# TonyLianLong/LLM-groundedDiffusion

Hardware: AMD Instinct MI355X
Metric: images/sec (50-step SD1.5 512^2, LMD+ guidance) (higher is better)
Workload: dtype fp16; 1 GPU; LMD+ stage 2, 4 cached 2-box layouts/GPU/step (lmd_v0.1 cache), 50 DDIM steps, 512x512, sd14_gligen (SD1.4+GLIGEN architecture, seeded random weights), VAE decodes included; per-box masks = box masks; mask_refinement=box, layouts_per_gpu=4, num_inference_steps=50, parallelism=dp1, rccl_ranks=1, lanes_per_gpu=4, gemm_tuning=throughput

## Files before the change

llm-groundeddiffusion_amd/csrc/gemm.hip:

```cpp
#include "common.h"
#include "../../include/lgd_hip.h"
#include <map>
#include <mutex>
#include <utility>
#include <stdlib.h>

namespace {

constexpr int BK = 64;
constexpr int LDS_LD = BK + 16;

struct GemmArgs {
  LgdGemmDesc d;
  int cin;
  int k_per_split;
  int group_m;
#ifdef LGD_GEMM_ABLATION
  int stagger;
#endif
};

__device__ __forceinline__ float4 ld_bias4(const float* p, int n) {
  return *reinterpret_cast<const float4*>(p + n);
}

__device__ __forceinline__ f32x4 rownorm4(const LgdGemmDesc& d, int m, int n_in, f32x4 v) {
  if (d.epi & LGD_EPI_ROWNORM) {
    const float2 st = *reinterpret_cast<const float2*>(d.rowstat + (long)m * 2);
    const float4 cs = *reinterpret_cast<const float4*>(d.colsum + n_in);
    v[0] = st.y * (v[0] - st.x * cs.x); v[1] = st.y * (v[1] - st.x * cs.y);
    v[2] = st.y * (v[2] - st.x * cs.z); v[3] = st.y * (v[3] - st.x * cs.w);
  }
  return v;
}

template <bool GEGLU>
__device__ __forceinline__ f32x4 epilogue_value4(const LgdGemmDesc& d, long r_off, int m, int n_out, f32x4 v, f32x4 g,
                                                 float4 bv, float4 bg, bool res_ready, half4_t res_pre) {
  v[0] += bv.x; v[1] += bv.y; v[2] += bv.z; v[3] += bv.w;
  if (GEGLU) {
    g[0] += bg.x; g[1] += bg.y; g[2] += bg.z; g[3] += bg.w;
#ifdef LGD_GEMM_ABLATION
    if (d.epi & (1 << 16)) {
#pragma unroll
      for (int r = 0; r < 4; ++r) v[r] = v[r] * g[r];
    } else
#endif
    {
      const f32x2_t g01 = gelu2_f((f32x2_t){g[0], g[1]}), g23 = gelu2_f((f32x2_t){g[2], g[3]});
      v[0] *= g01[0]; v[1] *= g01[1]; v[2] *= g23[0]; v[3] *= g23[1];
    }
  }
  const float alpha = d.alpha;
#pragma unroll
  for (int r = 0; r < 4; ++r) v[r] *= alpha;
  if (res_ready) {
#pragma unroll
    for (int r = 0; r < 4; ++r) v[r] += (float)res_pre[r];
  } else if (d.res) {
    if (d.epi & LGD_EPI_RES_F32) {
      const float* rp = reinterpret_cast<const float*>(d.res) + r_off + (long)m * d.ldr + n_out;
      float4 rv = *reinterpret_cast<const float4*>(rp);
      v[0] += rv.x; v[1] += rv.y; v[2] += rv.z; v[3] += rv.w;
    } else {
      const half_t* rp = reinterpret_cast<const half_t*>(d.res) + r_off + (long)m * d.ldr + n_out;
      half4_t rv = *reinterpret_cast<const half4_t*>(rp);
#pragma unroll
      for (int r = 0; r < 4; ++r) v[r] += (float)rv[r];
    }
  }
  return v;
}

template <bool GEGLU>
__device__ __forceinline__ void epilogue_store4(const LgdGemmDesc& d, long c_off, long r_off, int m,
                                                int n_out, f32x4 v, f32x4 g, float4 bv, float4 bg,
                                                bool res_ready = false,
                                                half4_t res_pre = (half4_t){0, 0, 0, 0}) {
  v = epilogue_value4<GEGLU>(d, r_off, m, n_out, v, g, bv, bg, res_ready, res_pre);
  if (d.epi & LGD_EPI_OUT_F32) {
    float* cp = reinterpret_cast<float*>(d.c) + c_off + (long)m * d.ldc + n_out;
    *reinterpret_cast<float4*>(cp) = make_float4(v[0], v[1], v[2], v[3]);
  } else {
    half_t* cp = reinterpret_cast<half_t*>(d.c) + c_off + (long)m * d.ldc + n_out;
    half4_t o;
#pragma unroll
    for (int r = 0; r < 4; ++r) o[r] = (half_t)v[r];
    *reinterpret_cast<half4_t*>(cp) = o;
  }
}

__device__ __forceinline__ float4 ld_bias_sum4(const LgdGemmDesc& d, int n) {
  float4 b = make_float4(0.f, 0.f, 0.f, 0.f);
  if (d.bias) b = ld_bias4(d.bias, n);
  if (d.bias2) {
    float4 b2 = ld_bias4(d.bias2, n);
    b.x += b2.x; b.y += b2.y; b.z += b2.z; b.w += b2.w;
  }
  return b;
}

template <int MI, int NI>
__device__ __forceinline__ void gemm_epilogue(const GemmArgs& ga, f32x4 (&acc)[NI][MI], int m0, int n0,
                                              int wm, int wn, int lane, int batch, int split,
                                              long c_off, long r_off, int* lds_flag = nullptr) {
  const LgdGemmDesc& d = ga.d;
  const int m_l = lane & 15;
  const int n_l = (lane >> 4) * 4;
  if (d.splits > 1) {
    float* ws = ga.d.ws + ((long)batch * d.splits + split) * (long)d.M * d.N;
#pragma unroll
    for (int mi = 0; mi < MI; ++mi) {
      int m = m0 + wm * 16 * MI + mi * 16 + m_l;
      if (m >= d.M) continue;
#pragma unroll
      for (int ni = 0; ni < NI; ++ni) {
        int n = n0 + wn * 16 * NI + ni * 16 + n_l;
        if (n >= d.N) continue;
        f32x4 v = acc[ni][mi];
        *reinterpret_cast<float4*>(ws + (long)m * d.N + n) = make_float4(v[0], v[1], v[2], v[3]);
      }
    }
    if (!d.cnt || !lds_flag) return;
    asm volatile("s_waitcnt vmcnt(0)" ::: "memory");
    __syncthreads();
    int32_t* cnt = d.cnt + (long)batch * gridDim.x + blockIdx.x;
    if (threadIdx.x == 0) {
      __builtin_amdgcn_fence(__ATOMIC_RELEASE, "agent");
      asm volatile("s_waitcnt vmcnt(0)" ::: "memory");
      *lds_flag = __hip_atomic_fetch_add(cnt, 1, __ATOMIC_RELAXED, __HIP_MEMORY_SCOPE_AGENT);
    }
    __syncthreads();
    if (*lds_flag != d.splits - 1) return;
    if (threadIdx.x == 0) {
      __builtin_amdgcn_fence(__ATOMIC_ACQUIRE, "agent");
      __hip_atomic_store(cnt, 0, __ATOMIC_RELAXED, __HIP_MEMORY_SCOPE_AGENT);
    }
    __syncthreads();
    const float* w0 = ga.d.ws + (long)batch * d.splits * (long)d.M * d.N;
#pragma unroll
    for (int mi = 0; mi < MI; ++mi) {
      const int m = m0 + wm * 16 * MI + mi * 16 + m_l;
#pragma unroll
      for (int ni = 0; ni < NI; ++ni) {
        const int n = n0 + wn * 16 * NI + ni * 16 + n_l;
        f32x4 v = {0.f, 0.f, 0.f, 0.f};
        if (m < d.M && n < d.N) {
          for (int s2 = 0; s2 < d.splits; ++s2) {
            const float4 t = *reinterpret_cast<const float4*>(w0 + (long)s2 * d.M * d.N + (long)m * d.N + n);
            v[0] += t.x; v[1] += t.y; v[2] += t.z; v[3] += t.w;
          }
        }
        acc[ni][mi] = v;
      }
    }
  }
  const bool geglu = d.epi & LGD_EPI_GEGLU;
  if (geglu) {
// ... 48 lines not shown
        const int m = m0 + wm * 16 * MI + mi * 16 + m_l;
        if (m < d.M)
          epilogue_store4<false>(d, c_off, r_off, m, n, rownorm4(d, m, n, acc[ni][mi]), acc[ni][mi], bv, bv, res16,
                                 res16 ? rpre[nj][mi] : (half4_t){0, 0, 0, 0});
      }
    }
  }
}

template <int MI, int NI, int WM, int WN, int STAGE_B, bool GEGLU, bool RES_PREFETCH>
__device__ __forceinline__ void gemm_epilogue_lds_generic(const GemmArgs& ga, f32x4 (&acc)[NI][MI], int m0, int n0, int wm,
                                                  int wn, int lane, int tid, long c_off, long r_off,
                                                  unsigned char* lds) {
  const LgdGemmDesc& d = ga.d;
  constexpr int NT = 64 * WM * WN;
  constexpr int BM = WM * 16 * MI, BN = WN * 16 * NI;
  constexpr int BN_OUT = GEGLU ? BN / 2 : BN;
  constexpr int NI_OUT = GEGLU ? NI / 2 : NI;
  constexpr int CROW = BN_OUT * 2 + 16;
  constexpr int R = (BM * CROW <= STAGE_B) ? 1 : ((BM / 2) * CROW <= STAGE_B) ? 2 : 4;
  static_assert(MI % R == 0 && (BM / R) * CROW <= STAGE_B, "staged rows must fit one ring stage");
  constexpr int MI_R = MI / R;
  constexpr int WROWS = 16 * MI_R;
  constexpr int RROWS = WM * WROWS;
  constexpr int CPR = BN_OUT / 8;
  const int m_l = lane & 15, n_l = (lane >> 4) * 4;
  const int n0_out = GEGLU ? n0 / 2 : n0;
  const int n_total_out = GEGLU ? d.N / 2 : d.N;
  const bool res16 = d.res && !(d.epi & LGD_EPI_RES_F32);
  half_t* cbase = reinterpret_cast<half_t*>(d.c) + c_off;
  float4 bv[NI_OUT], bg[NI_OUT];
  const bool rn = d.epi & LGD_EPI_ROWNORM;
  float4 cv[NI_OUT], cg[NI_OUT];
  float2 st[MI];
#pragma unroll
  for (int no = 0; no < NI_OUT; ++no) {
    const int n_out = n0_out + wn * 16 * NI_OUT + no * 16 + n_l;
    const int n_in = GEGLU ? n0 + wn * 16 * NI + no * 32 + n_l : n_out;
    bv[no] = make_float4(0.f, 0.f, 0.f, 0.f);
    bg[no] = bv[no];
    cv[no] = bv[no];
    cg[no] = bv[no];
#ifdef LGD_GEMM_ABLATION
    if (d.epi & (1 << 18)) continue;
#endif
    if (n_out < n_total_out) {
      bv[no] = ld_bias_sum4(d, n_in);
      if (GEGLU && d.bias) bg[no] = ld_bias4(d.bias, n_in + 16);
      if (rn) {
        cv[no] = *reinterpret_cast<const float4*>(d.colsum + n_in);
        if (GEGLU) cg[no] = *reinterpret_cast<const float4*>(d.colsum + n_in + 16);
      }
    }
  }
#pragma unroll
  for (int mi = 0; mi < MI; ++mi) {
    int m = m0 + wm * 16 * MI + mi * 16 + m_l;
    if (m >= d.M) m = d.M - 1;
    st[mi] = rn ? *reinterpret_cast<const float2*>(d.rowstat + (long)m * 2) : make_float2(0.f, 1.f);
  }
  auto rownorm = [&](f32x4 v, const float2 s2, const float4 c) {
    if (rn) {
      v[0] = s2.y * (v[0] - s2.x * c.x); v[1] = s2.y * (v[1] - s2.x * c.y);
      v[2] = s2.y * (v[2] - s2.x * c.z); v[3] = s2.y * (v[3] - s2.x * c.w);
    }
    return v;
  };
#pragma unroll
  for (int r = 0; r < R; ++r) {
    half4_t rpre[NI_OUT][MI_R];
    if (res16 && !GEGLU) {
      const half_t* rb = reinterpret_cast<const half_t*>(d.res) + r_off;
#pragma unroll
      for (int no = 0; no < NI_OUT; ++no) {
        int n = n0_out + wn * 16 * NI_OUT + no * 16 + n_l;
        if (n >= n_total_out) n = 0;
#pragma unroll
        for (int mj = 0; mj < MI_R; ++mj) {
          int m = m0 + wm * 16 * MI + (r * MI_R + mj) * 16 + m_l;
          if (m >= d.M) m = d.M - 1;
          rpre[no][mj] = *reinterpret_cast<const half4_t*>(rb + (long)m * d.ldr + n);
        }
      }
    }
#pragma unroll
    for (int no = 0; no < NI_OUT; ++no) {
      const int n_out = n0_out + wn * 16 * NI_OUT + no * 16 + n_l;
      const int nn = n_out < n_total_out ? n_out : 0;
#pragma unroll
      for (int mj = 0; mj < MI_R; ++mj) {
        const int mi = r * MI_R + mj;
        int m = m0 + wm * 16 * MI + mi * 16 + m_l;
        if (m >= d.M) m = d.M - 1;
        f32x4 v;
        if constexpr (GEGLU) {
          v = epilogue_value4<true>(d, r_off, m, nn, rownorm(acc[2 * no][mi], st[mi], cv[no]), rownorm(acc[2 * no + 1][mi], st[mi], cg[no]),
                                    bv[no], bg[no], false, (half4_t){0, 0, 0, 0});
        } else {
          v = epilogue_value4<false>(d, r_off, m, nn, rownorm(acc[no][mi], st[mi], cv[no]), acc[no][mi], bv[no], bv[no], res16,
                                     res16 ? rpre[no][mj] : (half4_t){0, 0, 0, 0});
        }
        half4_t o;
#pragma unroll
        for (int e = 0; e < 4; ++e) o[e] = (half_t)v[e];
        *reinterpret_cast<half4_t*>(lds + (wm * WROWS + mj * 16 + m_l) * CROW + (wn * 16 * NI_OUT + no * 16 + n_l) * 2) = o;
      }
    }
    asm volatile("s_waitcnt lgkmcnt(0)" ::: "memory");
    __builtin_amdgcn_s_barrier();
#pragma unroll
    for (int i = 0; i < (RROWS * CPR + NT - 1) / NT; ++i) {
      const int idx = tid + i * NT;
      const int row = idx / CPR, ch = idx - row * CPR;
      const int wr = row / WROWS;
      const int m = m0 + wr * 16 * MI + r * WROWS + (row - wr * WROWS), n = n0_out + ch * 8;
#ifdef LGD_GEMM_ABLATION
      if ((d.epi & (1 << 17)) && idx != 0) continue;
#endif
      if (idx < RROWS * CPR && m < d.M && n < n_total_out) {
        const uint4 val = *reinterpret_cast<const uint4*>(lds + row * CROW + ch * 16);
        *reinterpret_cast<uint4*>(cbase + (long)m * d.ldc + n) = val;
      }
    }
    if (r + 1 < R || !RES_PREFETCH) {
      asm volatile("s_waitcnt lgkmcnt(0)" ::: "memory");
      __builtin_amdgcn_s_barrier();
    }
  }
}

template <int MI, int NI, int WM, int WN, int STAGE_B, bool GEGLU, bool RES_PREFETCH, bool RES16, bool RN>
__device__ __forceinline__ void gemm_epilogue_lds(const GemmArgs& ga, f32x4 (&acc)[NI][MI], int m0, int n0, int wm,
                                                  int wn, int lane, int tid, long c_off, long r_off,
                                                  unsigned char* lds) {
  static_assert(!(GEGLU && RES16), "GEGLU outputs take no residual here");
  const LgdGemmDesc& d = ga.d;
  constexpr int NT = 64 * WM * WN;
  constexpr int BM = WM * 16 * MI, BN = WN * 16 * NI;
  constexpr int BN_OUT = GEGLU ? BN / 2 : BN;
  constexpr int NI_OUT = GEGLU ? NI / 2 : NI;
  constexpr int CROW = BN_OUT * 2 + 16;
  constexpr int R = (BM * CROW <= STAGE_B) ? 1 : ((BM / 2) * CROW <= STAGE_B) ? 2 : 4;
  static_assert(MI % R == 0 && (BM / R) * CROW <= STAGE_B, "staged rows must fit one ring stage");
  constexpr int MI_R = MI / R;
  constexpr int WROWS = 16 * MI_R;
  constexpr int RROWS = WM * WROWS;
  constexpr int CPR = BN_OUT / 8;
  const int m_l = lane & 15, n_l = (lane >> 4) * 4;
  const int n0_out = GEGLU ? n0 / 2 : n0;
  const int n_total_out = GEGLU ? d.N / 2 : d.N;
  half_t* cbase = reinterpret_cast<half_t*>(d.c) + c_off;
  const f32x2_t alpha2 = {d.alpha, d.alpha};
  constexpr bool LEAN = MI * NI >= 32;
  constexpr bool LEAN2 = MI * NI >= 32 && WN == 4;
  float4 bv[NI_OUT], bg[NI_OUT], cv[NI_OUT], cg[NI_OUT];
  int ncol[NI_OUT];
#pragma unroll
  for (int no = 0; no < NI_OUT; ++no) {
    const int n_out = n0_out + wn * 16 * NI_OUT + no * 16 + n_l;
    const int n_in = GEGLU ? n0 + wn * 16 * NI + no * 32 + n_l : n_out;
    const bool ok = n_out < n_total_out;
    ncol[no] = ok ? n_out : 0;
    bv[no] = make_float4(0.f, 0.f, 0.f, 0.f);
    bg[no] = bv[no];
    cv[no] = bv[no];
    cg[no] = bv[no];
#ifdef LGD_GEMM_ABLATION
    if (d.epi & (1 << 18)) continue;
#endif
    if (ok && !LEAN2) {
      bv[no] = ld_bias_sum4(d, n_in);
      if (GEGLU && d.bias) bg[no] = ld_bias4(d.bias, n_in + 16);
      if constexpr (RN && !LEAN) {
        cv[no] = *reinterpret_cast<const float4*>(d.colsum + n_in);
        if (GEGLU) cg[no] = *reinterpret_cast<const float4*>(d.colsum + n_in + 16);
      }
    }
  }
  int mrow[MI];
  float2 st[MI];
#pragma unroll
  for (int mi = 0; mi < MI; ++mi) {
    int m = m0 + wm * 16 * MI + mi * 16 + m_l;
    if (m >= d.M) m = d.M - 1;
    mrow[mi] = m;
    st[mi] = make_float2(0.f, 1.f);
    if constexpr (RN && !LEAN2) st[mi] = *reinterpret_cast<const float2*>(d.rowstat + (long)m * 2);
  }
  auto normed = [&](const f32x4& v, const float2 s2, const float4 c, const float4 b, f32x2_t& lo, f32x2_t& hi) {
    lo = (f32x2_t){v[0], v[1]};
    hi = (f32x2_t){v[2], v[3]};
    if constexpr (RN) {
      const f32x2_t mean = {s2.x, s2.x}, rstd = {s2.y, s2.y};
      lo = rstd * (lo - mean * (f32x2_t){c.x, c.y});
      hi = rstd * (hi - mean * (f32x2_t){c.z, c.w});
    }
    lo += (f32x2_t){b.x, b.y};
    hi += (f32x2_t){b.z, b.w};
  };
  unsigned char* lw = lds + (wm * WROWS + m_l) * CROW + (wn * 16 * NI_OUT + n_l) * 2;
#pragma unroll
  for (int r = 0; r < R; ++r) {
    if constexpr (RN && LEAN2) {
#pragma unroll
      for (int mj = 0; mj < MI_R; ++mj)
        st[r * MI_R + mj] = *reinterpret_cast<const float2*>(d.rowstat + (long)mrow[r * MI_R + mj] * 2);
    }
    half4_t rpre[NI_OUT][MI_R];
    if constexpr (RES16) {
      const half_t* rb = reinterpret_cast<const half_t*>(d.res) + r_off;
#pragma unroll
      for (int mj = 0; mj < MI_R; ++mj) {
        const half_t* rrow = rb + (long)mrow[r * MI_R + mj] * d.ldr;
#pragma unroll
        for (int no = 0; no < NI_OUT; ++no) {
          int nc = ncol[no];
          if constexpr (LEAN) {
            const int n_out = n0_out + wn * 16 * NI_OUT + no * 16 + n_l;
            nc = n_out < n_total_out ? n_out : 0;
          }
          rpre[no][mj] = *reinterpret_cast<const half4_t*>(rrow + nc);
        }
      }
    }
#pragma unroll
    for (int no = 0; no < NI_OUT; ++no) {
      if constexpr ((RN && LEAN) || LEAN2) {
        const int n_out = n0_out + wn * 16 * NI_OUT + no * 16 + n_l;
        const int n_in = GEGLU ? n0 + wn * 16 * NI + no * 32 + n_l : n_out;
        if (n_out < n_total_out) {
          if constexpr (RN) {
            cv[no] = *reinterpret_cast<const float4*>(d.colsum + n_in);
            if (GEGLU) cg[no] = *reinterpret_cast<const float4*>(d.colsum + n_in + 16);
          }
          if constexpr (LEAN2) {
            bv[no] = ld_bias_sum4(d, n_in);
            if (GEGLU && d.bias) bg[no] = ld_bias4(d.bias, n_in + 16);
          }
        }
      }
#pragma unroll
      for (int mj = 0; mj < MI_R; ++mj) {
        const int mi = r * MI_R + mj;
        f32x2_t lo, hi;
        if constexpr (GEGLU) {
          f32x2_t glo, ghi;
          normed(acc[2 * no][mi], st[mi], cv[no], bv[no], lo, hi);
          normed(acc[2 * no + 1][mi], st[mi], cg[no], bg[no], glo, ghi);
#ifdef LGD_GEMM_ABLATION
          if (d.epi & (1 << 16)) { lo *= glo; hi *= ghi; } else
#endif
          { lo *= gelu2_f(glo); hi *= gelu2_f(ghi); }
        } else {
          normed(acc[no][mi], st[mi], cv[no], bv[no], lo, hi);
        }
        lo *= alpha2;
        hi *= alpha2;
        if constexpr (RES16) {
          const half4_t rr = rpre[no][mj];
          lo += (f32x2_t){(float)rr[0], (float)rr[1]};
          hi += (f32x2_t){(float)rr[2], (float)rr[3]};
        }
        const half4_t o = {(half_t)lo[0], (half_t)lo[1], (half_t)hi[0], (half_t)hi[1]};
        *reinterpret_cast<half4_t*>(lw + mj * 16 * CROW + no * 32) = o;
      }
    }
    asm volatile("s_waitcnt lgkmcnt(0)" ::: "memory");
    __builtin_amdgcn_s_barrier();
#pragma unroll LEAN2 ? 1 : (RROWS * CPR + NT - 1) / NT
    for (int i = 0; i < (RROWS * CPR + NT - 1) / NT; ++i) {
      const int idx = tid + i * NT;
      const int row = idx / CPR, ch = idx - row * CPR;
      const int wr = row / WROWS;
      const int m = m0 + wr * 16 * MI + r * WROWS + (row - wr * WROWS), n = n0_out + ch * 8;
#ifdef LGD_GEMM_ABLATION
      if ((d.epi & (1 << 17)) && idx != 0) continue;
#endif
      if (idx < RROWS * CPR && m < d.M && n < n_total_out) {
        const uint4 val = *reinterpret_cast<const uint4*>(lds + row * CROW + ch * 16);
        *reinterpret_cast<uint4*>(cbase + (long)m * d.ldc + n) = val;
      }
    }
    if (r + 1 < R || !RES_PREFETCH) {
      asm volatile("s_waitcnt lgkmcnt(0)" ::: "memory");
      __builtin_amdgcn_s_barrier();
    }
  }
}

template <int MI, int NI>
__global__ __launch_bounds__(256) void gemm_kernel(const GemmArgs ga) {
  constexpr int BM = 32 * MI;
  constexpr int BN = 32 * NI;
  constexpr int A_IT = BM * 8 / 256;
  constexpr int B_IT = BN * 8 / 256;
  static_assert(A_IT >= 1 && B_IT >= 1, "tile too small");

  __shared__ __attribute__((aligned(16))) half_t smem[(BM + BN) * LDS_LD];
  half_t* As = smem;
  half_t* Bs = smem + BM * LDS_LD;

  const LgdGemmDesc& d = ga.d;
  const int tid = threadIdx.x;
  const int lane = tid & 63;
  const int wid = tid >> 6;
  const int wm = wid >> 1, wn = wid & 1;

// ... 903 lines not shown
  const int frow = lane & 15, fg = lane >> 4, fsw = (frow >> 1) & 7;
  const unsigned lds0 = (unsigned)(uintptr_t)smem;
  unsigned a_ad0 = lds0 + (grp * 16 * MH + frow) * 128 + ((0 + fg) ^ fsw) * 16;
  unsigned a_ad1 = lds0 + (grp * 16 * MH + frow) * 128 + ((4 + fg) ^ fsw) * 16;
  unsigned b_ad0 = lds0 + OFF_B0 + (wn * 16 + frow) * 128 + ((0 + fg) ^ fsw) * 16;
  unsigned b_ad1 = lds0 + OFF_B0 + (wn * 16 + frow) * 128 + ((4 + fg) ^ fsw) * 16;
  using seqA = std::make_integer_sequence<int, MH>;
  using seqB0 = std::make_integer_sequence<int, NI0>;
  using seqB1 = std::make_integer_sequence<int, NI1>;

  f32x4 acc[NI][MI];
  half8_t af[2][MH], bf0[2][NI0], bf1[2][NI1];
  if constexpr (ABL & 2) {
#pragma unroll
    for (int kk = 0; kk < 2; ++kk) {
#pragma unroll
      for (int i = 0; i < MH; ++i) af[kk][i] = (half8_t){1, 1, 1, 1, 1, 1, 1, 1};
#pragma unroll
      for (int i = 0; i < NI0; ++i) bf0[kk][i] = (half8_t){1, 1, 1, 1, 1, 1, 1, 1};
#pragma unroll
      for (int i = 0; i < NI1; ++i) bf1[kk][i] = (half8_t){1, 1, 1, 1, 1, 1, 1, 1};
    }
  }

#define LGD_PH_MMA(BF, NB, NOFF, MOFF)                                                                              \
  {                                                                                                                 \
    asm volatile("s_waitcnt lgkmcnt(0)" ::: "memory");                                                              \
    __builtin_amdgcn_sched_barrier(0);                                                                              \
    if constexpr (!(ABL & 32)) __builtin_amdgcn_s_setprio(1);                                                       \
    _Pragma("unroll") for (int kk = 0; kk < 2; ++kk)                                                                \
      _Pragma("unroll") for (int ni = 0; ni < NB; ++ni)                                                             \
        _Pragma("unroll") for (int mi = 0; mi < MH; ++mi)                                                           \
          if constexpr (ABL & 4) asm volatile("" : "+v"(acc[NOFF + ni][MOFF + mi]) : "v"(BF[kk][ni]), "v"(af[kk][mi]));                \
          else acc[NOFF + ni][MOFF + mi] = __builtin_amdgcn_mfma_f32_16x16x32_f16(BF[kk][ni], af[kk][mi], acc[NOFF + ni][MOFF + mi], 0, 0, 0); \
    if constexpr (!(ABL & 32)) __builtin_amdgcn_s_setprio(0);                                                       \
    __builtin_amdgcn_sched_barrier(0);                                                                              \
  }
#define LGD_PH_BAR()                        \
  {                                         \
    __builtin_amdgcn_sched_barrier(0);      \
    __builtin_amdgcn_s_barrier();           \
    __builtin_amdgcn_sched_barrier(0);      \
  }

  if (nk > 0) {
    {
      unsigned sa, sw; int tap;
      k_pos(0, sa, sw, tap);
      dma_b(0, 0, true, sw, false);
      dma_a(0, 0, true, sa, tap, false);
      dma_b(1, 0, true, sw, false);
      dma_a(1, 0, true, sa, tap, false);
      k_pos(1, sa, sw, tap);
      dma_b(0, STAGE_B, nk > 1, sw, false);
      dma_a(0, STAGE_B, nk > 1, sa, tap, false);
    }
#pragma unroll
    for (int ni = 0; ni < NI; ++ni)
#pragma unroll
      for (int mi = 0; mi < MI; ++mi) acc[ni][mi] = (f32x4){0.f, 0.f, 0.f, 0.f};
    asm volatile("s_waitcnt vmcnt(%0)" ::"n"(T_DMA) : "memory");
    LGD_PH_BAR();
    if (grp == 1 && !(ABL & 64)) LGD_PH_BAR();
    unsigned so_cur = 0, so_nxt = STAGE_B;
    int sdelta = STAGE_B;
    for (int kt = 0; kt < nk; ++kt) {
      unsigned sa1, sw1, sa2, sw2; int tap1, tap2;
      k_pos(kt + 1, sa1, sw1, tap1);
      k_pos(kt + 2, sa2, sw2, tap2);
      const bool live1 = kt + 1 < nk, live2 = kt + 2 < nk;
      if constexpr (!(ABL & 2)) lds_read_frags<0, 64 * 128>(bf0[0], b_ad0, seqB0{});
      if constexpr (!(ABL & 2)) lds_read_frags<0, 64 * 128>(bf0[1], b_ad1, seqB0{});
      if constexpr (!(ABL & 2)) lds_read_frags<0, 16 * 128>(af[0], a_ad0, seqA{});
      if constexpr (!(ABL & 2)) lds_read_frags<0, 16 * 128>(af[1], a_ad1, seqA{});
      dma_b(1, so_nxt, live1, sw1);
      asm volatile("s_waitcnt vmcnt(%0)" ::"n"(T_DMA) : "memory");
      LGD_PH_BAR();
      LGD_PH_MMA(bf0, NI0, 0, 0);
      LGD_PH_BAR();
      if constexpr (!(ABL & 2)) lds_read_frags<BQ0_B, 64 * 128>(bf1[0], b_ad0, seqB1{});
      if constexpr (!(ABL & 2)) lds_read_frags<BQ0_B, 64 * 128>(bf1[1], b_ad1, seqB1{});
      dma_a(1, so_nxt, live1, sa1, tap1);
      asm volatile("s_waitcnt vmcnt(%0)" ::"n"(T_DMA) : "memory");
      LGD_PH_BAR();
      LGD_PH_MMA(bf1, NI1, NI0, 0);
      LGD_PH_BAR();
      if constexpr (!(ABL & 2)) lds_read_frags<OFF_A1, 16 * 128>(af[0], a_ad0, seqA{});
      if constexpr (!(ABL & 2)) lds_read_frags<OFF_A1, 16 * 128>(af[1], a_ad1, seqA{});
      dma_b(0, so_cur, live2, sw2);
      LGD_PH_BAR();
      LGD_PH_MMA(bf1, NI1, NI0, MH);
      LGD_PH_BAR();
      dma_a(0, so_cur, live2, sa2, tap2);
      asm volatile("s_waitcnt vmcnt(%0)" ::"n"(T_DMA) : "memory");
      LGD_PH_BAR();
      LGD_PH_MMA(bf0, NI0, 0, MH);
      LGD_PH_BAR();
      a_ad0 += sdelta; a_ad1 += sdelta; b_ad0 += sdelta; b_ad1 += sdelta;
      sdelta = -sdelta;
      const unsigned t = so_cur; so_cur = so_nxt; so_nxt = t;
    }
    if (grp == 0 && !(ABL & 64)) LGD_PH_BAR();
    asm volatile("s_waitcnt vmcnt(0) lgkmcnt(0)" ::: "memory");
    LGD_PH_BAR();
  }
  else {
#pragma unroll
    for (int ni = 0; ni < NI; ++ni)
#pragma unroll
      for (int mi = 0; mi < MI; ++mi) acc[ni][mi] = (f32x4){0.f, 0.f, 0.f, 0.f};
  }
#undef LGD_PH_MMA
#undef LGD_PH_BAR

  if constexpr (ABL & 16) {
#pragma unroll
    for (int ni = 0; ni < NI; ++ni)
#pragma unroll
      for (int mi = 0; mi < MI; ++mi) asm volatile("" ::"v"(acc[ni][mi]));
    return;
  }
  if (d.splits > 1) {
    const int m_l = lane & 15, n_l = (lane >> 4) * 4;
    float* ws = d.ws + ((long)batch * d.splits + split) * (long)d.M * d.N;
#pragma unroll
    for (int mi = 0; mi < MI; ++mi) {
      const int m = m0 + grp * 16 * MI + mi * 16 + m_l;
      if (m >= d.M) continue;
#pragma unroll
      for (int ni = 0; ni < NI; ++ni) {
        const int n = n0 + wn * 16 * NI + ni * 16 + n_l;
        if (n >= d.N) continue;
        const f32x4 v = acc[ni][mi];
        *reinterpret_cast<float4*>(ws + (long)m * d.N + n) = make_float4(v[0], v[1], v[2], v[3]);
      }
    }
    return;
  }
#define LGD_EPI_LDS(G, RS, RNORM) \
  gemm_epilogue_lds<MI, NI, WM, WN, (MI * NI > 32 ? STAGE_B : 2 * STAGE_B), G, true, RS, RNORM>(ga, acc, m0, n0, grp, wn, lane, tid, c_off, r_off, lds)
  const bool rn_ = d.epi & LGD_EPI_ROWNORM;
  if (d.epi & LGD_EPI_GEGLU) {
    if constexpr (NI % 2 == 0) {
      if (rn_) LGD_EPI_LDS(true, false, true); else LGD_EPI_LDS(true, false, false);
    }
  } else if (d.res) {
    if (rn_) LGD_EPI_LDS(false, true, true); else LGD_EPI_LDS(false, true, false);
  } else {
    if (rn_) LGD_EPI_LDS(false, false, true); else LGD_EPI_LDS(false, false, false);
  }
#undef LGD_EPI_LDS
}

__global__ __launch_bounds__(256) void splitk_reduce_kernel(const GemmArgs ga) {
  const LgdGemmDesc& d = ga.d;
  const bool geglu = d.epi & LGD_EPI_GEGLU;
  const int n_out_cols = geglu ? d.N / 2 : d.N;
  const long groups_per_row = n_out_cols / 4;
  const long total = (long)d.M * groups_per_row;
  const int batch = blockIdx.z;
  const int b_o = batch / d.nb_i, b_i = batch - b_o * d.nb_i;
  const long c_off = b_o * d.c_bs_o + b_i * d.c_bs_i;
  const long r_off = b_o * d.r_bs_o + b_i * d.r_bs_i;
  const float* ws = d.ws + (long)batch * d.splits * (long)d.M * d.N;
  for (long idx = blockIdx.x * 256L + threadIdx.x; idx < total; idx += (long)gridDim.x * 256L) {
    int m = (int)(idx / groups_per_row);
    int gcol = (int)(idx - (long)m * groups_per_row) * 4;
    int n_in = geglu ? (gcol / 16) * 32 + (gcol % 16) : gcol;
    f32x4 v = {0.f, 0.f, 0.f, 0.f}, g = {0.f, 0.f, 0.f, 0.f};
    for (int s = 0; s < d.splits; ++s) {
      const float* p = ws + (long)s * d.M * d.N + (long)m * d.N + n_in;
      float4 t = *reinterpret_cast<const float4*>(p);
      v[0] += t.x; v[1] += t.y; v[2] += t.z; v[3] += t.w;
      if (geglu) {
        float4 u = *reinterpret_cast<const float4*>(p + 16);
        g[0] += u.x; g[1] += u.y; g[2] += u.z; g[3] += u.w;
      }
    }
    const float4 bv = ld_bias_sum4(d, n_in);
    v = rownorm4(d, m, n_in, v);
    if (geglu) {
      float4 bg = make_float4(0.f, 0.f, 0.f, 0.f);
      if (d.bias) bg = ld_bias4(d.bias, n_in + 16);
      epilogue_store4<true>(d, c_off, r_off, m, gcol, v, rownorm4(d, m, n_in + 16, g), bv, bg);
    } else {
      epilogue_store4<false>(d, c_off, r_off, m, gcol, v, g, bv, bv);
    }
  }
}

enum GemmLoop : int {
  LOOP_REG,
  LOOP_DMA,
  LOOP_DMA8,
  LOOP_PIPE,
  LOOP_PHASE,
};
enum : unsigned {
  TILE_GEGLU = 1,
  TILE_PLAIN = 2,
  TILE_ONE_SPLIT = 4,
  TILE_LDS_EPI = 8,
  TILE_CONV_SAME = 16,
  TILE_CNT = 32,
};
struct GemmTile {
  int code;
  GemmLoop loop;
  int bm, bn;
  unsigned flags;
};
constexpr unsigned TILE_STD = TILE_GEGLU | TILE_CNT;
constexpr GemmTile GEMM_TILES[] = {
    {1, LOOP_REG, 128, 128, TILE_STD},   {2, LOOP_REG, 128, 64, TILE_STD},     {3, LOOP_REG, 64, 128, TILE_STD},
    {4, LOOP_REG, 64, 64, TILE_STD},     {5, LOOP_REG, 32, 128, TILE_STD},     {6, LOOP_REG, 128, 160, TILE_CNT},
    {7, LOOP_REG, 64, 160, TILE_CNT},
    {17, LOOP_DMA, 128, 128, TILE_STD},  {18, LOOP_DMA, 128, 64, TILE_STD},    {19, LOOP_DMA, 64, 128, TILE_STD},
    {20, LOOP_DMA, 64, 64, TILE_STD},    {21, LOOP_DMA, 32, 128, TILE_STD},    {22, LOOP_DMA, 128, 160, TILE_CNT},
    {23, LOOP_DMA, 64, 160, TILE_CNT},
    {25, LOOP_DMA8, 256, 320, TILE_CNT}, {26, LOOP_DMA8, 256, 128, TILE_STD},
    {33, LOOP_PIPE, 256, 160, TILE_CNT}, {34, LOOP_PIPE, 256, 128, TILE_STD}, {35, LOOP_PIPE, 256, 64, TILE_STD},
    {37, LOOP_PIPE, 128, 160, TILE_CNT}, {38, LOOP_PIPE, 128, 128, TILE_STD}, {39, LOOP_PIPE, 128, 64, TILE_STD},
    {40, LOOP_PIPE, 64, 160, TILE_CNT},  {41, LOOP_PIPE, 64, 128, TILE_STD},  {42, LOOP_PIPE, 64, 64, TILE_STD},
    {44, LOOP_PIPE, 256, 256, TILE_GEGLU | TILE_PLAIN | TILE_ONE_SPLIT | TILE_LDS_EPI},
    {45, LOOP_PIPE, 128, 128, TILE_STD | TILE_PLAIN},
    {46, LOOP_PHASE, 256, 256, TILE_GEGLU | TILE_LDS_EPI | TILE_CONV_SAME},
    {47, LOOP_PHASE, 256, 320, TILE_LDS_EPI | TILE_CONV_SAME},
};

const GemmTile* gemm_check(const LgdGemmDesc& desc, GemmArgs& ga) {
  ga.d = desc;
  LgdGemmDesc& d = ga.d;
  if (d.M <= 0 || d.N <= 0 || d.K <= 0) return nullptr;
  if (d.taps != 1 && d.taps != 9) return nullptr;
  ga.cin = d.c0 + d.c1;
  if (d.K != d.taps * ga.cin) return nullptr;
  if ((d.c0 % 8) || (d.c1 % 8) || (d.N % 4) || (d.ldw % 8) || (d.lda0 % 8) || (d.lda1 % 8) ||
      (d.ldc % 4))
    return nullptr;
  if (d.c1 > 0 && !d.a1) return nullptr;
  if (d.res && (d.ldr % 4)) return nullptr;
  if (d.nb_o < 1) d.nb_o = 1;
  if (d.nb_i < 1) d.nb_i = 1;
  if (d.splits < 1) d.splits = 1;
  const bool geglu = d.epi & LGD_EPI_GEGLU;
  if (geglu && (d.N % 32)) return nullptr;
  if (d.splits > 1 && !d.ws) return nullptr;
  if ((d.epi & LGD_EPI_ROWNORM) && (!d.rowstat || !d.colsum || d.taps != 1 || d.nb_o * d.nb_i != 1 || d.c1 > 0))
    return nullptr;
  int ktiles = (d.K + BK - 1) / BK;
  int tps = (ktiles + d.splits - 1) / d.splits;
  ga.k_per_split = tps * BK;
  d.splits = (ktiles + tps - 1) / tps;

  int code = d.tile;
  if (code == 0) {
    long batches = (long)d.nb_o * d.nb_i * d.splits;
    auto wgs = [&](int bm, int bn) {
      return batches * ((d.M + bm - 1) / bm) * ((d.N + bn - 1) / bn);
    };
    if (d.M <= 32) code = 21;
    else if (!geglu && d.N % 160 == 0 && wgs(128, 160) >= 384) code = 22;
    else if (!geglu && d.N % 160 == 0 && wgs(64, 160) >= 256) code = 23;
    else if (wgs(128, 128) >= 384 && d.N % 128 == 0) code = 17;
    else if (wgs(64, 128) >= 256 && d.N % 128 == 0) code = 19;
    else code = 20;
  }
  const GemmTile* t = nullptr;
  for (const GemmTile& e : GEMM_TILES)
    if (e.code == code) t = &e;
  if (!t) return nullptr;
  const unsigned f = t->flags;
  if (geglu && !(f & TILE_GEGLU)) return nullptr;
  if (t->loop == LOOP_DMA8 && (d.K % BK)) return nullptr;
  if ((t->loop == LOOP_PIPE || t->loop == LOOP_PHASE) && ((d.K % BK) || (ga.cin % BK) || (d.c0 % BK))) return nullptr;
  if ((f & TILE_PLAIN) && (d.taps != 1 || d.c1 > 0)) return nullptr;
  if (t->loop == LOOP_PHASE) {
    if (d.c1 > 0 || d.nb_o * d.nb_i != 1) return nullptr;
    if (((long)d.M + 2L * d.win + 2) * d.lda0 * 2 + 2L * d.K >= (1L << 31) || (long)d.N * d.ldw * 2 >= (1L << 31))
      return nullptr;
  }
  if ((f & TILE_CONV_SAME) && d.taps == 9 && (d.stride != 1 || d.ups != 0 || d.hin != d.hout || d.win != d.wout))
    return nullptr;
  if ((f & TILE_ONE_SPLIT) && d.splits != 1) return nullptr;
  if ((f & TILE_LDS_EPI) && d.splits == 1) {
    const long c_off_max = (long)(d.nb_o - 1) * d.c_bs_o + (long)(d.nb_i - 1) * d.c_bs_i;
    if ((d.epi & LGD_EPI_OUT_F32) || (d.N & 7) || (d.ldc & 7) || (c_off_max & 7) || (d.c_bs_o & 7) || (d.c_bs_i & 7) ||
        (reinterpret_cast<uintptr_t>(d.c) & 15) || (d.res && (d.epi & (LGD_EPI_RES_F32 | LGD_EPI_GEGLU))))
      return nullptr;
  }
  if (d.splits > 1 && d.cnt && !(f & TILE_CNT)) return nullptr;
  return t;
}

using GemmKernel = void (*)(GemmArgs);

int lds_kernel(GemmKernel kern, int smem, int threads, long* resident = nullptr) {
  static std::mutex mu;
  static std::map<std::pair<GemmKernel, int>, long> ready;
  int dev = 0;
  if (hipGetDevice(&dev) != hipSuccess) return LGD_ERR_LAUNCH;
  std::lock_guard<std::mutex> lock(mu);
  auto it = ready.find({kern, dev});
  if (it == ready.end()) {
    if (hipFuncSetAttribute(reinterpret_cast<const void*>(kern), hipFuncAttributeMaxDynamicSharedMemorySize, smem) !=
        hipSuccess)
      return LGD_ERR_LAUNCH;
    it = ready.emplace(std::make_pair(kern, dev), -1L).first;
  }
  if (resident) {
    if (it->second < 0) {
      int per_cu = 0, cus = 0;
      if (hipDeviceGetAttribute(&cus, hipDeviceAttributeMultiprocessorCount, dev) != hipSuccess ||
          hipOccupancyMaxActiveBlocksPerMultiprocessor(&per_cu, reinterpret_cast<const void*>(kern), threads, smem) !=
              hipSuccess)
        return LGD_ERR_LAUNCH;
      it->second = (long)(cus / 8) * 8 * (per_cu > 0 ? per_cu : 1);
    }
    *resident = it->second;
  }
  return LGD_OK;
}

template <int MI, int NI, int WM = 2>
int launch_gemm(const GemmArgs& ga, hipStream_t st, bool dma) {
  constexpr int BM = WM * 16 * MI, BN = 32 * NI;
  const LgdGemmDesc& d = ga.d;
  long tiles = (long)((d.M + BM - 1) / BM) * ((d.N + BN - 1) / BN);
  dim3 grid((unsigned)tiles, 1, (unsigned)(d.nb_o * d.nb_i * d.splits));
  if constexpr (WM == 2) {
    if (dma) hipLaunchKernelGGL((gemm_dma_kernel<MI, NI, 2>), grid, dim3(256), 0, st, ga);
    else hipLaunchKernelGGL((gemm_kernel<MI, NI>), grid, dim3(256), 0, st, ga);
  } else {
    hipLaunchKernelGGL((gemm_dma_kernel<MI, NI, WM>), grid, dim3(128 * WM), 0, st, ga);
  }
  return lgd_check_launch();
}

template <int MI, int NI, int WM, int WN, int NS, bool CM>
int launch_gemm_pipe_cm(const GemmArgs& ga, hipStream_t st) {
  constexpr int BM = WM * 16 * MI, BN = WN * 16 * NI;
  constexpr int SMEM = NS * (BM + BN) * BK * 2;
  constexpr int THREADS = 64 * WM * WN;
  constexpr bool HAS_PERSIST = !CM && !(MI == 4 && NI == 5) && NS != 2;
  const LgdGemmDesc& d = ga.d;
  long tiles = (long)((d.M + BM - 1) / BM) * ((d.N + BN - 1) / BN);
  GemmKernel kern = &gemm_pipe_kernel<MI, NI, WM, WN, NS, CM>;
  long resident = 0;
  if constexpr (HAS_PERSIST) {
    static const bool persist_on = [] { const char* e = getenv("LGD_GEMM_PERSIST"); return !(e && e[0] == '0'); }();
    if (persist_on)
      if (int rc = lds_kernel(&gemm_pipe_kernel<MI, NI, WM, WN, NS, false, true>, SMEM, THREADS, &resident)) return rc;
  }
  const bool persist = resident > 0 && d.nb_o * d.nb_i * d.splits == 1 && tiles > resident && d.K <= 10 * BK && d.taps == 1;
  dim3 grid((unsigned)(persist ? resident : tiles), 1, (unsigned)(d.nb_o * d.nb_i * d.splits));
  if constexpr (HAS_PERSIST)
    if (persist) kern = &gemm_pipe_kernel<MI, NI, WM, WN, NS, false, true>;
#ifdef LGD_GEMM_ABLATION
  static const int abl = [] { const char* e = getenv("LGD_GEMM_ABL"); return e ? atoi(e) : 0; }();
  if (abl) {
    switch (abl) {
      case 1: kern = &gemm_pipe_kernel<MI, NI, WM, WN, NS, CM, false, 1>; break;
      case 2: kern = &gemm_pipe_kernel<MI, NI, WM, WN, NS, CM, false, 2>; break;
      case 3: kern = &gemm_pipe_kernel<MI, NI, WM, WN, NS, CM, false, 3>; break;
      case 4: kern = &gemm_pipe_kernel<MI, NI, WM, WN, NS, CM, false, 4>; break;
      case 6: kern = &gemm_pipe_kernel<MI, NI, WM, WN, NS, CM, false, 6>; break;
      case 8: kern = &gemm_pipe_kernel<MI, NI, WM, WN, NS, CM, false, 8>; break;
      case 11: kern = &gemm_pipe_kernel<MI, NI, WM, WN, NS, CM, false, 11>; break;
      case 16: kern = &gemm_pipe_kernel<MI, NI, WM, WN, NS, CM, false, 16>; break;
      case 17: kern = &gemm_pipe_kernel<MI, NI, WM, WN, NS, CM, false, 17>; break;
      case 20: kern = &gemm_pipe_kernel<MI, NI, WM, WN, NS, CM, false, 20>; break;
      default: return lgd_check_launch();
    }
  }
#endif
  if (int rc = lds_kernel(kern, SMEM, THREADS)) return rc;
  hipLaunchKernelGGL(kern, grid, dim3(THREADS), SMEM, st, ga);
  return lgd_check_launch();
}

template <int MI, int NI, int WM, int WN, int NS>
int launch_gemm_pipe(const GemmArgs& ga, hipStream_t st) {
  const LgdGemmDesc& d = ga.d;
  static const int no_cm = [] { const char* e = getenv("LGD_GEMM_NO_CM"); return (e && e[0] == '1') ? 1 : 0; }();
  if constexpr (NS != 2) {
    if (d.taps == 9 && d.stride == 1 && d.ups == 0 && d.c1 == 0 && !no_cm)
      return launch_gemm_pipe_cm<MI, NI, WM, WN, NS, true>(ga, st);
  }
  return launch_gemm_pipe_cm<MI, NI, WM, WN, NS, false>(ga, st);
}

template <int MI, int NI>
int launch_gemm_phase(const GemmArgs& ga, hipStream_t st) {
  constexpr int BM = 32 * MI, BN = 64 * NI;
  constexpr int SMEM = 2 * (BM + BN) * BK * 2;
  const LgdGemmDesc& d = ga.d;
  const bool conv = d.taps == 9;
  long tiles = (long)((d.M + BM - 1) / BM) * ((d.N + BN - 1) / BN);
  dim3 grid((unsigned)tiles, 1, (unsigned)(d.nb_o * d.nb_i * d.splits));
  GemmKernel kern = conv ? &gemm_phase_kernel<MI, NI, true> : &gemm_phase_kernel<MI, NI, false>;
#ifdef LGD_GEMM_ABLATION
  static const int abl = [] { const char* e = getenv("LGD_GEMM_ABL"); return e ? atoi(e) : 0; }();
  if (abl) {
#define LGD_PH_ABL(A) case A: kern = conv ? &gemm_phase_kernel<MI, NI, true, A> : &gemm_phase_kernel<MI, NI, false, A>; break;
    switch (abl) {
      LGD_PH_ABL(1) LGD_PH_ABL(2) LGD_PH_ABL(3) LGD_PH_ABL(4) LGD_PH_ABL(6) LGD_PH_ABL(16) LGD_PH_ABL(17) LGD_PH_ABL(20) LGD_PH_ABL(32) LGD_PH_ABL(64) LGD_PH_ABL(96)
      default: return lgd_check_launch();
    }
#undef LGD_PH_ABL
  }
#endif
  if (int rc = lds_kernel(kern, SMEM, 512)) return rc;
  hipLaunchKernelGGL(kern, grid, dim3(512), SMEM, st, ga);
  return lgd_check_launch();
}

int launch_tile(const GemmTile& t, const GemmArgs& ga, hipStream_t st) {
  const bool dma = t.loop == LOOP_DMA && ga.d.K % BK == 0;
  switch (t.code) {
    case 33: return launch_gemm_pipe<4, 5, 4, 2, 3>(ga, st);
    case 34: return launch_gemm_pipe<4, 4, 4, 2, 3>(ga, st);
    case 35: return launch_gemm_pipe<4, 2, 4, 2, 4>(ga, st);
    case 37: return launch_gemm_pipe<2, 5, 4, 2, 4>(ga, st);
    case 38: return launch_gemm_pipe<2, 4, 4, 2, 4>(ga, st);
    case 39: return launch_gemm_pipe<2, 2, 4, 2, 5>(ga, st);
    case 40: return launch_gemm_pipe<1, 5, 4, 2, 5>(ga, st);
    case 41: return launch_gemm_pipe<1, 4, 4, 2, 5>(ga, st);
    case 42: return launch_gemm_pipe<1, 2, 4, 2, 6>(ga, st);
    case 44: return launch_gemm_pipe<4, 8, 4, 2, 2>(ga, st);
    case 45: return launch_gemm_pipe<2, 4, 4, 2, 2>(ga, st);
    case 46: return launch_gemm_phase<8, 4>(ga, st);
    case 47: return launch_gemm_phase<8, 5>(ga, st);
    case 1: case 17: return launch_gemm<4, 4>(ga, st, dma);
    case 2: case 18: return launch_gemm<4, 2>(ga, st, dma);
    case 3: case 19: return launch_gemm<2, 4>(ga, st, dma);
    case 4: case 20: return launch_gemm<2, 2>(ga, st, dma);
    case 5: case 21: return launch_gemm<1, 4>(ga, st, dma);
    case 6: case 22: return launch_gemm<4, 5>(ga, st, dma);
    case 7: case 23: return launch_gemm<2, 5>(ga, st, dma);
    case 25: return launch_gemm<4, 10, 4>(ga, st, true);
    case 26: return launch_gemm<4, 4, 4>(ga, st, true);
  }
  return LGD_ERR_ARG;
}

}

extern "C" int lgd_abi_version(void) { return LGD_ABI_VERSION; }

extern "C" int lgd_gemm_check(const LgdGemmDesc* desc) {
  GemmArgs ga;
  return desc && gemm_check(*desc, ga) ? LGD_OK : LGD_ERR_ARG;
}

extern "C" int lgd_gemm_f16(const LgdGemmDesc* desc, void* stream) {
  (void)hipGetLastError();
  GemmArgs ga;
  const GemmTile* t = desc ? gemm_check(*desc, ga) : nullptr;
  if (!t) return LGD_ERR_ARG;
  const LgdGemmDesc& d = ga.d;
  hipStream_t st = reinterpret_cast<hipStream_t>(stream);
#ifdef LGD_GEMM_ABLATION
  { const char* e = getenv("LGD_GEMM_STAGGER"); ga.stagger = e ? atoi(e) : 0; }
#endif
  {
    static const int forced = [] { const char* e = getenv("LGD_GEMM_GROUP_M"); return e ? atoi(e) : 0; }();
    ga.group_m = 1;
    const long w_bytes = (long)d.N * d.K * 2;
    if (d.taps == 1 && d.nb_o * d.nb_i == 1 && w_bytes > (5L << 19)) {
      long g = (3L << 20) / (256L * d.K * 2);
      ga.group_m = forced > 0 ? forced : (int)(g < 1 ? 1 : g > 8 ? 8 : g);
    }
  }
  int rc = launch_tile(*t, ga, st);
  if (rc || d.splits == 1 || d.cnt) return rc;
  int n_out = (d.epi & LGD_EPI_GEGLU) ? d.N / 2 : d.N;
  long total = (long)d.M * (n_out / 4);
  int blocks = (int)((total + 255) / 256);
  if (blocks > 2048) blocks = 2048;
  dim3 grid(blocks, 1, d.nb_o * d.nb_i);
  hipLaunchKernelGGL(splitk_reduce_kernel, grid, dim3(256), 0, st, ga);
  return lgd_check_launch();
}
```

Before: 1.786 images/s.

## Add opt-in 4-wave phase GEMM kernel with interleaved MFMA/LDS/DMA schedule

Adds a 256-thread, 4-wave variant of the phase GEMM kernel in which each wave computes an 8xNI MFMA tile. LDS fragment reads and buffer-to-LDS DMA loads are interleaved between MFMAs under explicit scheduling barriers, aiming to hide load latency with fewer waves. The kernel is selected only when LGD_PHASE_LOOP=wave4 is set. Separately, the LDS epilogue's lean bias path is widened to any tile with MI*NI >= 64, which changes the default epilogue for large tiles.

```diff
diff --git a/llm-groundeddiffusion_amd/csrc/gemm.hip b/llm-groundeddiffusion_amd/csrc/gemm.hip
--- a/llm-groundeddiffusion_amd/csrc/gemm.hip
+++ b/llm-groundeddiffusion_amd/csrc/gemm.hip
@@ -4,6 +4,8 @@
 #include <mutex>
 #include <utility>
 #include <stdlib.h>
+#include <string.h>
+#include <type_traits>
 
 namespace {
 
@@ -358,7 +360,7 @@
   half_t* cbase = reinterpret_cast<half_t*>(d.c) + c_off;
   const f32x2_t alpha2 = {d.alpha, d.alpha};
   constexpr bool LEAN = MI * NI >= 32;
-  constexpr bool LEAN2 = MI * NI >= 32 && WN == 4;
+  constexpr bool LEAN2 = MI * NI >= 32 && (WN == 4 || MI * NI >= 64);
   float4 bv[NI_OUT], bg[NI_OUT], cv[NI_OUT], cg[NI_OUT];
   int ncol[NI_OUT];
 #pragma unroll
@@ -1568,6 +1570,275 @@
 #undef LGD_EPI_LDS
 }
 
+template <class F, int... I>
+__device__ __forceinline__ void static_for(std::integer_sequence<int, I...>, F&& f) {
+  (f(std::integral_constant<int, I>{}), ...);
+}
+template <int NA, int NB>
+__device__ __forceinline__ void wait_lds_set(half8_t (&a)[NA], half8_t (&b)[NB]) {
+  asm volatile("s_waitcnt lgkmcnt(0)" ::: "memory");
+#pragma unroll
+  for (int i = 0; i < NA; ++i) asm volatile("" : "+v"(a[i]));
+#pragma unroll
+  for (int i = 0; i < NB; ++i) asm volatile("" : "+v"(b[i]));
+}
+__device__ __forceinline__ void dma_piece(const half_t* base, unsigned nrec, unsigned char* dst, unsigned voff, unsigned soff) {
+  const __amdgpu_buffer_rsrc_t rs = __builtin_amdgcn_make_buffer_rsrc(const_cast<half_t*>(base), 0, nrec, 0x00020000);
+  __builtin_amdgcn_raw_ptr_buffer_load_lds(rs, (lds_ptr_t)dst, 16, voff, soff, 0, 0);
+}
+__device__ __forceinline__ void sched_fence() { __builtin_amdgcn_sched_barrier(0); }
+template <bool OFF>
+__device__ __forceinline__ void mfma_step(f32x4& c, const half8_t& b, const half8_t& a) {
+  if constexpr (OFF) asm volatile("" : "+v"(c) : "v"(b), "v"(a));
+  else c = __builtin_amdgcn_mfma_f32_16x16x32_f16(b, a, c, 0, 0, 0);
+}
+
+template <int NI, bool CM, int ABL = 0>
+__global__ __launch_bounds__(256, 1) void gemm_phase4_kernel(const GemmArgs ga) {
+  constexpr int MI = 8, WM = 2, WN = 2;
+  constexpr int BM = WM * 16 * MI, BN = WN * 16 * NI;
+  constexpr int OFF_B = BM * BK * 2;
+  constexpr int STAGE_B = (BM + BN) * BK * 2;
+  static_assert(2 * STAGE_B <= 160 * 1024, "LDS");
+  constexpr int PA = BM / 32, PB = BN / 32;
+  constexpr int T_DMA = PA + PB;
+  constexpr int NMF = MI * NI;
+  constexpr int NRD = MI + NI;
+  static_assert(2 * NRD <= NMF && 2 * T_DMA <= NMF, "one filler per MFMA gap");
+  constexpr unsigned OOB = 0x80000000u;
+  constexpr unsigned NREC = 0x80000000u;
+
+  extern __shared__ __attribute__((aligned(1024))) half_t smem[];
+  unsigned char* lds = reinterpret_cast<unsigned char*>(smem);
+
+  const LgdGemmDesc& d = ga.d;
+  const int tid = threadIdx.x;
+  const int lane = tid & 63;
+  const int wid = __builtin_amdgcn_readfirstlane(tid >> 6);
+  const int wr = wid >> 1, wc = wid & 1;
+
+  const int n_tiles_n = (d.N + BN - 1) / BN;
+  const int total_tiles = ((d.M + BM - 1) / BM) * n_tiles_n;
+  int m0, n0;
+  {
+    const int q = total_tiles >> 3, r = total_tiles & 7;
+    const int xcd = blockIdx.x & 7, idx = blockIdx.x >> 3;
+    const int bid = (xcd < r ? xcd * (q + 1) : r * (q + 1) + (xcd - r) * q) + idx;
+    int tile_m, tile_n;
+    if (ga.group_m > 1) {
+      const int per_group = ga.group_m * n_tiles_n;
+      const int g = bid / per_group, in = bid - g * per_group;
+      const int n_tiles_m = total_tiles / n_tiles_n;
+      int rows = n_tiles_m - g * ga.group_m;
+      if (rows > ga.group_m) rows = ga.group_m;
+      tile_n = in / rows;
+      tile_m = g * ga.group_m + (in - tile_n * rows);
+    } else {
+      tile_m = bid / n_tiles_n;
+      tile_n = bid - tile_m * n_tiles_n;
+    }
+    m0 = __builtin_amdgcn_readfirstlane(tile_m * BM);
+    n0 = __builtin_amdgcn_readfirstlane(tile_n * BN);
+  }
+  const int split = blockIdx.z;
+  const int k_beg = split * ga.k_per_split;
+  int k_end = k_beg + ga.k_per_split;
+  if (k_end > d.K) k_end = d.K;
+  const int nk = __builtin_amdgcn_readfirstlane((k_end - k_beg) / BK);
+  const int cin = ga.cin;
+
+  const int lrow = lane >> 3;
+  const int kseg = (lane & 7) ^ ((((wid & 1) << 2) + (lrow >> 1)) & 7);
+  const unsigned lda2 = (unsigned)d.lda0 * 2u, ldw2 = (unsigned)d.ldw * 2u;
+  const int prow = wid * 8 + lrow;
+  const half_t* a_base = reinterpret_cast<const half_t*>(d.a0) - (CM ? (long)(d.win + 1) * d.lda0 : 0L);
+  const half_t* w_base = reinterpret_cast<const half_t*>(d.w);
+  const unsigned voffA = (unsigned)(m0 + prow) * lda2 + kseg * 16;
+  const unsigned voffB = (unsigned)(n0 + prow) * ldw2 + kseg * 16;
+  unsigned amask[PA / 2];
+#pragma unroll
+  for (int u = 0; u < PA / 2; ++u) amask[u] = 0u;
+#pragma unroll
+  for (int u = 0; u < PA; ++u) {
+    const int m = m0 + u * 32 + prow;
+    if (m >= d.M) continue;
+    if (CM) {
+      const int ox = m % d.wout, oy = (m / d.wout) % d.hout;
+#pragma unroll
+      for (int t = 0; t < 9; ++t) {
+        const int iy = oy + t / 3 - 1, ix = ox + t % 3 - 1;
+        if (iy >= 0 && ix >= 0 && iy < d.hin && ix < d.win) amask[u >> 1] |= 1u << (9 * (u & 1) + t);
+      }
+    } else {
+      amask[u >> 1] |= 1u << (9 * (u & 1));
+    }
+  }
+  unsigned bmask = 0;
+#pragma unroll
+  for (int u = 0; u < PB; ++u)
+    if (n0 + u * 32 + prow < d.N) bmask |= 1u << u;
+
+  const int t0 = k_beg / BK;
+  auto k_pos = [&](int kt, unsigned& sa, unsigned& sw, int& tap) {
+    if (CM) {
+      const int t = t0 + kt, ch = __builtin_amdgcn_readfirstlane(t / 9);
+      tap = t - ch * 9;
+      const int ky = tap / 3, kx = tap - ky * 3;
+      sa = (unsigned)(ky * d.win + kx) * lda2 + (unsigned)ch * (BK * 2);
+      sw = (unsigned)(tap * cin + ch * BK) * 2u;
+    } else {
+      tap = 0;
+      sa = sw = (unsigned)(k_beg + kt * BK) * 2u;
+    }
+  };
+  struct Src {
+    unsigned sa, sw, nrec;
+    int tap;
+  };
+  auto src = [&](int kt, bool live) {
+    Src s;
+    k_pos(kt, s.sa, s.sw, s.tap);
+    s.nrec = live ? NREC : 0u;
+    return s;
+  };
+  auto dma = [&](auto pc, unsigned so, const Src& s) {
+    constexpr int P = decltype(pc)::value;
+    if constexpr (P < PA) {
+      const unsigned vo = ((amask[P >> 1] >> (9 * (P & 1) + s.tap)) & 1u) ? voffA : OOB;
+      dma_piece(a_base, s.nrec, lds + so + P * 4096 + wid * 1024, vo, s.sa + (unsigned)(P * 32) * lda2);
+    } else {
+      constexpr int U = P - PA;
+      const unsigned vo = ((bmask >> U) & 1u) ? voffB : OOB;
+      dma_piece(w_base, s.nrec, lds + so + OFF_B + U * 4096 + wid * 1024, vo, s.sw + (unsigned)(U * 32) * ldw2);
+    }
+  };
+  using seqD = std::make_integer_sequence<int, T_DMA>;
+
+  const int frow = lane & 15, fg = lane >> 4, fsw = (frow >> 1) & 7;
+  const unsigned lds0 = (unsigned)(uintptr_t)smem;
+  unsigned a_ad[2], b_ad[2];
+#pragma unroll
+  for (int kk = 0; kk < 2; ++kk) {
+    a_ad[kk] = lds0 + (wr * 16 * MI + frow) * 128 + ((4 * kk + fg) ^ fsw) * 16;
+    b_ad[kk] = lds0 + OFF_B + (wc * 16 * NI + frow) * 128 + ((4 * kk + fg) ^ fsw) * 16;
+  }
+
+  f32x4 acc[NI][MI];
+  half8_t af[2][MI], bf[2][NI];
+  if constexpr (ABL & 2) {
+#pragma unroll
+    for (int kk = 0; kk < 2; ++kk) {
+#pragma unroll
+      for (int i = 0; i < MI; ++i) af[kk][i] = (half8_t){1, 1, 1, 1, 1, 1, 1, 1};
+#pragma unroll
+      for (int i = 0; i < NI; ++i) bf[kk][i] = (half8_t){1, 1, 1, 1, 1, 1, 1, 1};
+    }
+  }
+  auto rd = [&](auto kc, auto rc) {
+    constexpr int KK = decltype(kc)::value, R = decltype(rc)::value;
+    if constexpr (ABL & 2) return;
+    else if constexpr (R < MI) lds_read128<R * 16 * 128>(af[KK][R], a_ad[KK]);
+    else lds_read128<(R - MI) * 16 * 128>(bf[KK][R - MI], b_ad[KK]);
+  };
+  auto wait_set = [&](auto kc) { wait_lds_set(af[decltype(kc)::value], bf[decltype(kc)::value]); };
+  auto half = [&](auto kc, unsigned so, const Src& s) {
+    constexpr int KK = decltype(kc)::value;
+    static_for(std::make_integer_sequence<int, NMF>{}, [&](auto gc) {
+      constexpr int G = decltype(gc)::value, NJ = G / MI, MJ = G % MI;
+      mfma_step<(ABL & 4) != 0>(acc[NJ][MJ], bf[KK][NJ], af[KK][MJ]);
+      if constexpr (G % 2 == 0 && G / 2 < NRD) rd(std::integral_constant<int, 1 - KK>{}, std::integral_constant<int, G / 2>{});
+      if constexpr (KK == 1 && !(ABL & 1) && G % 2 == 1 && G / 2 < T_DMA) dma(std::integral_constant<int, G / 2>{}, so, s);
+      sched_fence();
+    });
+  };
+#define LGD_PH4_BAR()                       \
+  {                                         \
+    __builtin_amdgcn_sched_barrier(0);      \
+    __builtin_amdgcn_s_barrier();           \
+    __builtin_amdgcn_sched_barrier(0);      \
+  }
+  constexpr std::integral_constant<int, 0> K0{};
+  constexpr std::integral_constant<int, 1> K1{};
+
+  if (nk > 0) {
+    {
+      const Src s0 = src(0, true), s1 = src(1, nk > 1);
+      static_for(seqD{}, [&](auto pc) { dma(pc, 0, s0); });
+      static_for(seqD{}, [&](auto pc) { dma(pc, STAGE_B, s1); });
+    }
+#pragma unroll
+    for (int ni = 0; ni < NI; ++ni)
+#pragma unroll
+      for (int mi = 0; mi < MI; ++mi) acc[ni][mi] = (f32x4){0.f, 0.f, 0.f, 0.f};
+    asm volatile("s_waitcnt vmcnt(%0)" ::"n"(T_DMA) : "memory");
+    LGD_PH4_BAR();
+    static_for(std::make_integer_sequence<int, NRD>{}, [&](auto rc) { rd(K0, rc); });
+    unsigned so_cur = 0;
+    int sdelta = STAGE_B;
+    for (int kt = 0; kt < nk; ++kt) {
+      const Src s2 = src(kt + 2, kt + 2 < nk);
+      wait_set(K0);
+      __builtin_amdgcn_sched_barrier(0);
+      half(K0, so_cur, s2);
+      asm volatile("s_waitcnt vmcnt(0)" ::: "memory");
+      wait_set(K1);
+      LGD_PH4_BAR();
+      a_ad[0] += sdelta; b_ad[0] += sdelta;
+      half(K1, so_cur, s2);
+      a_ad[1] += sdelta; b_ad[1] += sdelta;
+      sdelta = -sdelta;
+      so_cur ^= (unsigned)STAGE_B;
+    }
+    asm volatile("s_waitcnt vmcnt(0)" ::: "memory");
+    wait_set(K0);
+    LGD_PH4_BAR();
+  } else {
+#pragma unroll
+    for (int ni = 0; ni < NI; ++ni)
+#pragma unroll
+      for (int mi = 0; mi < MI; ++mi) acc[ni][mi] = (f32x4){0.f, 0.f, 0.f, 0.f};
+  }
+#undef LGD_PH4_BAR
+
+  if constexpr (ABL & 16) {
+#pragma unroll
+    for (int ni = 0; ni < NI; ++ni)
+#pragma unroll
+      for (int mi = 0; mi < MI; ++mi) asm volatile("" ::"v"(acc[ni][mi]));
+    return;
+  }
+  if (d.splits > 1) {
+    const int m_l = lane & 15, n_l = (lane >> 4) * 4;
+    float* ws = d.ws + (long)split * d.M * d.N;
+#pragma unroll
+    for (int mi = 0; mi < MI; ++mi) {
+      const int m = m0 + wr * 16 * MI + mi * 16 + m_l;
+      if (m >= d.M) continue;
+#pragma unroll
+      for (int ni = 0; ni < NI; ++ni) {
+        const int n = n0 + wc * 16 * NI + ni * 16 + n_l;
+        if (n >= d.N) continue;
+        const f32x4 v = acc[ni][mi];
+        *reinterpret_cast<float4*>(ws + (long)m * d.N + n) = make_float4(v[0], v[1], v[2], v[3]);
+      }
+    }
+    return;
+  }
+#define LGD_EPI_LDS(G, RS, RNORM) \
+  gemm_epilogue_lds<MI, NI, WM, WN, (NI > 8 ? STAGE_B : 2 * STAGE_B), G, true, RS, RNORM>(ga, acc, m0, n0, wr, wc, lane, tid, 0L, 0L, lds)
+  const bool rn_ = d.epi & LGD_EPI_ROWNORM;
+  if (d.epi & LGD_EPI_GEGLU) {
+    if constexpr (NI % 4 == 0) {
+      if (rn_) LGD_EPI_LDS(true, false, true); else LGD_EPI_LDS(true, false, false);
+    }
+  } else if (d.res) {
+    if (rn_) LGD_EPI_LDS(false, true, true); else LGD_EPI_LDS(false, true, false);
+  } else {
+    if (rn_) LGD_EPI_LDS(false, false, true); else LGD_EPI_LDS(false, false, false);
+  }
+#undef LGD_EPI_LDS
+}
+
 __global__ __launch_bounds__(256) void splitk_reduce_kernel(const GemmArgs ga) {
   const LgdGemmDesc& d = ga.d;
   const bool geglu = d.epi & LGD_EPI_GEGLU;
@@ -1810,24 +2081,39 @@
 int launch_gemm_phase(const GemmArgs& ga, hipStream_t st) {
   constexpr int BM = 32 * MI, BN = 64 * NI;
   constexpr int SMEM = 2 * (BM + BN) * BK * 2;
+  constexpr bool HAS4 = NI == 4;
   const LgdGemmDesc& d = ga.d;
   const bool conv = d.taps == 9;
   long tiles = (long)((d.M + BM - 1) / BM) * ((d.N + BN - 1) / BN);
   dim3 grid((unsigned)tiles, 1, (unsigned)(d.nb_o * d.nb_i * d.splits));
+  static const bool wave4 = [] { const char* e = getenv("LGD_PHASE_LOOP"); return e && strcmp(e, "wave4") == 0; }();
+  const bool four = HAS4 && wave4;
+  const int threads = four ? 256 : 512;
   GemmKernel kern = conv ? &gemm_phase_kernel<MI, NI, true> : &gemm_phase_kernel<MI, NI, false>;
+  if constexpr (HAS4)
+    if (four) kern = conv ? &gemm_phase4_kernel<2 * NI, true> : &gemm_phase4_kernel<2 * NI, false>;
 #ifdef LGD_GEMM_ABLATION
   static const int abl = [] { const char* e = getenv("LGD_GEMM_ABL"); return e ? atoi(e) : 0; }();
   if (abl) {
 #define LGD_PH_ABL(A) case A: kern = conv ? &gemm_phase_kernel<MI, NI, true, A> : &gemm_phase_kernel<MI, NI, false, A>; break;
-    switch (abl) {
-      LGD_PH_ABL(1) LGD_PH_ABL(2) LGD_PH_ABL(3) LGD_PH_ABL(4) LGD_PH_ABL(6) LGD_PH_ABL(16) LGD_PH_ABL(17) LGD_PH_ABL(20) LGD_PH_ABL(32) LGD_PH_ABL(64) LGD_PH_ABL(96)
-      default: return lgd_check_launch();
+#define LGD_PH4_ABL(A) case A: kern = conv ? &gemm_phase4_kernel<2 * NI, true, A> : &gemm_phase4_kernel<2 * NI, false, A>; break;
+    if (!four) {
+      switch (abl) {
+        LGD_PH_ABL(1) LGD_PH_ABL(2) LGD_PH_ABL(3) LGD_PH_ABL(4) LGD_PH_ABL(6) LGD_PH_ABL(16) LGD_PH_ABL(17) LGD_PH_ABL(20) LGD_PH_ABL(32) LGD_PH_ABL(64) LGD_PH_ABL(96)
+        default: return lgd_check_launch();
+      }
+    } else if constexpr (HAS4) {
+      switch (abl) {
+        LGD_PH4_ABL(1) LGD_PH4_ABL(2) LGD_PH4_ABL(3) LGD_PH4_ABL(4) LGD_PH4_ABL(6) LGD_PH4_ABL(16) LGD_PH4_ABL(17) LGD_PH4_ABL(20)
+        default: return lgd_check_launch();
+      }
     }
 #undef LGD_PH_ABL
+#undef LGD_PH4_ABL
   }
 #endif
-  if (int rc = lds_kernel(kern, SMEM, 512)) return rc;
-  hipLaunchKernelGGL(kern, grid, dim3(512), SMEM, st, ga);
+  if (int rc = lds_kernel(kern, SMEM, threads)) return rc;
+  hipLaunchKernelGGL(kern, grid, dim3(threads), SMEM, st, ga);
   return lgd_check_launch();
 }
 
```

Result: no change. 1.783 images/s, median of 2 (-0.2%).
